# lizaibeim/mmla-audio

Measured on AMD Instinct MI355X. Metric: audio clips/sec (MFCC→logits) at 1/2/4/8 MI355X; MFCC max-abs-err vs librosa, higher is better.
Workload: dtype f16x3+f32

## Files before the change

mmla_audio_amd/csrc/context.cpp:

```cpp
#include <algorithm>
#include <cstdarg>
#include <cstdio>
#include <cstdlib>

#include "internal.h"

using namespace mmla;

namespace mmla __attribute__((visibility("hidden"))) {

int fail(mmla_ctx* c, int code, const char* fmt, ...) {
  char buf[512];
  va_list ap;
  va_start(ap, fmt);
  vsnprintf(buf, sizeof(buf), fmt, ap);
  va_end(ap);
  if (c) c->err = buf;
  return code;
}

static hipEvent_t prof_event(mmla_ctx* c) {
  if (!c->prof_pool.empty()) {
    hipEvent_t e = c->prof_pool.back();
    c->prof_pool.pop_back();
// ... 105 lines not shown
                      side ? "trailing" : "leading", side ? i : g - i);
    }
  }
  return MMLA_OK;
}

int finish(mmla_ctx* c, bool dev) {
  HIPCHK(c, hipGetLastError());
  bool guarded = false;
  for (size_t g : c->ws_guard) guarded |= g != 0;
  if (!dev || guarded) HIPCHK(c, hipStreamSynchronize(c->stream));
  if (guarded) return ws_check_guards(c);
  return MMLA_OK;
}

constexpr double kOdBytesPerClip = 3.0 * 128 * 151 * 32 * 4 + 128 * 151 * 3 + 128 * 151 * 4 +
                                   19 * 128 * 4 + 512 * 4 + 64;
constexpr double kSiBytesPerClip = 4.0 * 256 * 32 * 4 + 256 * 39 * 4 + 8 * 128 * 4 + 512 * 4 +
                                   1024 * 4 + 64;

int64_t microbatch(mmla_ctx* c, bool od) {
  const int64_t user = od ? c->od_mb : c->si_mb;
  if (user > 0) return user;
  const int64_t cap = od ? c->od_mb_cap : c->si_mb_cap;
  size_t fr = 0, tot = 0;
  if (hipMemGetInfo(&fr, &tot) != hipSuccess) {
    (void)hipGetLastError();
    return cap;
  }
  double held = 0;
  for (size_t i = 0; i < c->ws_size.size(); ++i)
// ... 17 lines not shown
    {"MMLA_NO_SIFIN", &mmla_ctx::sifin, nullptr},
    {"MMLA_NO_SIPAIR", &mmla_ctx::sipair, nullptr},
    {"MMLA_NO_SICHAIN", &mmla_ctx::sichain, nullptr},
    {"MMLA_NO_LSTM_SPLIT", &mmla_ctx::lstm_split, nullptr},
    {"MMLA_LSTM_SPLIT_MAX", nullptr, &mmla_ctx::lstm_split_max},
    {"MMLA_DEBUG_LSTM_SPIN", nullptr, &mmla_ctx::lstm_spin},
    {"MMLA_DEBUG_TRACE_GUARD", nullptr, &mmla_ctx::debug_trace_guard},
    {"MMLA_NO_SIPAD", &mmla_ctx::si_pad_feat, nullptr},
    {"MMLA_NO_ODU", &mmla_ctx::odu, nullptr},
    {"MMLA_NO_ODW", &mmla_ctx::odw, nullptr},
    {"MMLA_NO_VADW", &mmla_ctx::vadw, nullptr},
    {"MMLA_VADW", nullptr, &mmla_ctx::vadw_all},
    {"MMLA_RB_TILE", &mmla_ctx::rbs, nullptr},
    {"MMLA_NO_RBS_W1L", &mmla_ctx::rbs_w1l, nullptr},
    {"MMLA_NO_RBS_TAILPAIR", &mmla_ctx::rbs_tailpair, nullptr},
    {"MMLA_NO_PIN_OUT", &mmla_ctx::pin_small, nullptr},
};

extern "C" {

int mmla_abi_version(void) { return MMLA_ABI_VERSION; }

int mmla_create(int device, mmla_ctx** out) {
  if (!out) return MMLA_E_INVALID;
  *out = nullptr;
  int ndev = 0;
  if (hipGetDeviceCount(&ndev) != hipSuccess || ndev == 0) return MMLA_E_HIP;
  if (device < 0 || device >= ndev) return MMLA_E_INVALID;
  if (hipSetDevice(device) != hipSuccess) return MMLA_E_HIP;
  mmla_ctx* c = new mmla_ctx();
// ... 190 lines not shown
```

mmla_audio_amd/csrc/internal.h:

```cpp
#pragma once
#include <hip/hip_runtime.h>

#include <cstdint>
#include <cstring>
#include <string>
#include <vector>

#include "../../include/mmla.h"
#include "nr.h"
#include "od_fe.h"
#include "mix.h"
#include "si_fe.h"
#include "ssim.h"
#include "vad.h"

namespace mmla __attribute__((visibility("hidden"))) {

constexpr int OD_H = 128, OD_W = 151, OD_PIX = OD_H * OD_W;
constexpr int OD_IMG = OD_PIX * 3;
constexpr int SI_T = 256, SI_D = 39;
constexpr int SI_NEED_SAMPLES = 160 * 259 + 400;
constexpr int CH[9] = {32, 32, 32, 64, 64, 64, 128, 128, 128};
constexpr bool POOL[9] = {true, false, false, true, false, false, true, false, false};

// ... 99 lines not shown
  int debug_trace_guard = 0;
  int precision = MMLA_PREC_F16X3;
  bool siu = true;
  bool sipu = true;
  bool sifin = true;
  bool sipair = true;
  bool sichain = true;
  bool si_pad_feat = true;
  bool odu = true;
  bool odw = true;
  bool vadw = true;
  int vadw_all = 0;
  bool rbs = true;
  bool rbs_w1l = true;
  bool rbs_tailpair = true;
  bool lstm_split = true;
  int lstm_split_max = 128;
  int lstm_spin = 0;
  int* range_dev = nullptr;
  int* range_host = nullptr;
  bool pin_small = true;
  int* range_map = nullptr;
  int* range_map_dev = nullptr;
  char* pin_out = nullptr;
  char* pin_out_dev = nullptr;
  char* pin_in = nullptr;
  int64_t lstm_split_reruns = 0;
  int64_t range_reruns = 0;
  bool od_f32_only = false, si_f32_only = false;
  bool si_base_f16_bad = false;
// ... 124 lines not shown
  int* timeout = nullptr;
  bool h3() const { return prec == MMLA_PREC_F16X3; }
};
inline Arith unguarded(const mmla_ctx* c) { return Arith{c->precision, c->lstm_split}; }

struct OdGate {
  const int32_t* lens = nullptr;
  int clip_len = -1;
  uint8_t* silent = nullptr;
  const float* ssim = nullptr;
  float ssim_threshold = 0.0f;
};

int run_od_net(mmla_ctx* c, const Arith& ar, const uint8_t* img_u8, const float* img_f32, int64_t n,
               float* probs, int32_t* argmax, OdGate gate = OdGate(), int stop = -1,
               const float** tap = nullptr, int64_t* tap_n = nullptr);
int run_si_net(mmla_ctx* c, const Arith& ar, const float* x, int64_t n, float* probs, int32_t* argmax,
               const uint8_t* silent, int ldx = SI_D, int stop = -1, const float** tap = nullptr,
               int64_t* tap_n = nullptr);

}
```

mmla_audio_amd/csrc/net_runners.cpp:

```cpp
#include <algorithm>

#include "conv.h"
#include "conv_h3.h"
#include "internal.h"
#include "nets.h"
#include "odu.h"
#include "resblk.h"
#include "siu.h"

using namespace mmla;

namespace {

ConvArgs conv_args(const ConvW& w, const float* x, float* y, int n, int h, int wd, int stride,
                   const BnW* bn, int pro, int epi, const float* res) {
  ConvArgs a{};
  a.x = x;
  a.wt = w.wt;
  a.bias = w.bias;
  a.scale = bn ? bn->scale : nullptr;
  a.shift = bn ? bn->shift : nullptr;
  a.res = res;
  a.y = y;
  a.n = n;
// ... 152 lines not shown
    k.path = OD_STRIPS;
    k.w1_lds = c->rbs_w1l && !POOL[b];
    k.tail_pair = c->rbs_tailpair && POOL[b];
  } else if (tiles_ok(B, POOL[b])) {
    k.path = OD_TILES;
  } else if (c->odu && odu_ok(B, POOL[b], h, w)) {
    k.path = OD_ODU;
    k.strips = c->odw && odu_two_strips(h, w, B.ca.cin, B.ca.cout, POOL[b]) ? 2 : 1;
  }
  k.stem = b == 0 && stop != 0 && (k.path == OD_STRIPS || k.path == OD_TILES);
  return k;
}

ResBlkArgs resblk_args(const ResUnitW& B, bool pool, bool fused, const float* x, float* y, int64_t n,
                       int h, int w, int* range_flag, const ConvW* stem, const uint8_t* img_u8,
                       const float* img_f32) {
  ResBlkArgs r{};
  r.x = x;
  r.y = y;
  r.w1h = fused ? B.ca.fh : B.ca.wh;
  r.w1l = fused ? B.ca.fl : B.ca.wl;
  r.b1 = B.ca.bias;
  r.u1 = B.ca.unscale();
  r.s1 = B.bn_in.scale;
  r.t1 = B.bn_in.shift;
  r.w2h = fused ? B.cb.fh : B.cb.wh;
  r.w2l = fused ? B.cb.fl : B.cb.wl;
  r.b2 = B.cb.bias;
  r.u2 = B.cb.unscale();
  r.s2 = B.bn_mid.scale;
  r.t2 = B.bn_mid.shift;
  if (pool) {
    r.wsh = fused ? B.sc.fh : B.sc.wh;
    r.wsl = fused ? B.sc.fl : B.sc.wl;
    r.bs = B.sc.bias;
    r.us = B.sc.unscale();
  }
  if (stem) {
    r.x = nullptr;
    r.img8 = img_u8;
    r.imgf = img_u8 ? nullptr : img_f32;
    r.wst = stem->wt;
    r.bst = stem->bias;
    r.ldst = stem->cout_pad;
  }
  r.n = (int)n;
  r.h = h;
  r.w = w;
  r.range_flag = range_flag;
  return r;
}

OduArgs odu_args(const ResUnitW& B, bool pool, const float* x, float* y, int64_t n, int* range_flag) {
  OduArgs o{};
  o.x = x;
// ... 43 lines not shown
    CHK(conv_spatial(c, ar, B.cb, T1, T2, n, h, w, &B.bn_mid, PRO_BN_ELU, EPI_BIAS, nullptr, true, 0, &B.sc,
                     X));
    std::swap(T1, T2);
  } else {
    CHK(conv_spatial(c, ar, B.cb, T1, T2, n, h, w, &B.bn_mid, PRO_BN_ELU, EPI_BIAS, nullptr, true));
    CHK(conv_run(c, conv_args(B.sc, X, T1, n, h, w, 2, nullptr, PRO_NONE, EPI_ADD, T2)));
  }
  *out = T1;
  return MMLA_OK;
}

}

namespace mmla __attribute__((visibility("hidden"))) {

int run_od_net(mmla_ctx* c, const Arith& ar, const uint8_t* img_u8, const float* img_f32, int64_t n,
               float* probs, int32_t* argmax, OdGate gate, int stop, const float** tap, int64_t* tap_n) {
  const OdNet& W = c->od;
  const size_t big = (size_t)n * OD_PIX * 32;
  float *X, *T1, *T2, *SEQ, *H;
  CHK(ws_floats(c, S_X, big, &X));
  CHK(ws_floats(c, S_T1, big, &T1));
  CHK(ws_floats(c, S_T2, big, &T2));
  CHK(ws_floats(c, S_SEQ, (size_t)n * 19 * 128, &SEQ));
  CHK(ws_floats(c, S_HOUT, (size_t)n * 512, &H));
  const double stem_flops = 2.0 * n * OD_PIX * 3 * 16;
  const OdChoice first = od_choose(c, ar, W.blk[0], 0, OD_H, OD_W, stop);
  if (!first.stem)
    LAUNCH(c, MMLA_STAGE_GLUE, stem_flops,
           od_stem_launch(img_u8, img_f32, n * OD_PIX, W.stem.cout_pad, W.stem.wt, W.stem.bias, X,
                          c->stream));
  int h = OD_H, w = OD_W;
  if (stop == 0) {
    *tap = X;
    *tap_n = n * OD_PIX * 16;
    return MMLA_OK;
  }
  for (int b = 0; b < 9; ++b) {
    const ResUnitW& B = W.blk[b];
    const bool pool = POOL[b];
    const OdChoice k = b == 0 ? first : od_choose(c, ar, B, b, h, w, stop);
    const double flops = od_block_flops(B, pool, n, h, w) + (k.stem ? stem_flops : 0.0);
    float* out = T1;
    switch (k.path) {
      case OD_STRIPS:
      case OD_TILES: {
        const bool tiles = k.path == OD_TILES;
        const ResBlkArgs r = resblk_args(B, pool, tiles, X, T1, n, h, w, ar.range,
                                         k.stem ? &W.stem : nullptr, img_u8, img_f32);
        LAUNCH(c, MMLA_STAGE_CONV, flops,
               tiles ? resblk_launch(r, B.ca.cin, B.ca.cout, pool, c->stream)
                     : rbs_launch(r, B.ca.cin, B.ca.cout, pool, k.w1_lds, k.tail_pair, c->stream));
        break;
      }
      case OD_ODU: {
        const OduArgs o = odu_args(B, pool, X, T1, n, ar.range);
        LAUNCH(c, MMLA_STAGE_CONV, flops,
               odu_launch(o, h, w, B.ca.cin, B.ca.cout, pool, k.strips, c->stream));
        break;
      }
      case OD_PAIR:
        CHK(od_block_pair(c, ar, B, pool, (int)n, h, w, X, T1, T2, &out));
        break;
    }
// ... 213 lines not shown
```

mmla_audio_amd/csrc/od_fe.h:

```cpp
#pragma once
#include <hip/hip_runtime.h>
#include <stdint.h>

struct OdFeTables {
  int mel_start[128];
  int mel_cnt[128];
  float mel_w[128][10];
  uint16_t a1[16][2][2][64][8];
  uint16_t a2[13][2][2][64][8];
  int mel_bt_bin0[8], mel_bt_nk[8], mel_bt_frag[8];
  int mel_unit[16];
  float mel_a[64][64];
  uint16_t zero16;
};

struct OdFeArgs {
  const int16_t* pcm;
  const float* pcm_f32;
  int64_t clip_stride;
  const int32_t* lens;
  int32_t clip_len;
  const OdFeTables* tables;
  float* db;
  float* norm;
  float* zcr;
  uint8_t* img;
  int* range_flag;
};

void od_fe_build_tables(OdFeTables* t);
bool od_fe_tables_ok(const OdFeTables& t);
hipError_t od_fe_launch(const OdFeArgs& a, int64_t n_clips, hipStream_t stream);
```

mmla_audio_amd/csrc/od_fe.hip:

```cpp
#include "common.h"
#include "od_fe.h"

#include <algorithm>
#include <cstdlib>
#include <cstring>
#include <type_traits>
#include <utility>

namespace {

constexpr int N_FFT = 400;
constexpr int HOP = 160;
constexpr int CLIP = 24000;
constexpr int NF = 151;
constexpr int NMEL = 128;
namespace v3 {

typedef float f32x16 __attribute__((ext_vector_type(16)));
typedef _Float16 f16x8 __attribute__((ext_vector_type(8)));
typedef uint16_t us2 __attribute__((ext_vector_type(2)));

constexpr int NWV = 16;
constexpr int NTH = 64 * NWV;
constexpr int TF = 32;
// ... 99 lines not shown
MMLA_DEV void for_tiles(F&& f, std::integer_sequence<int, I...>) {
  (f(tile_c<I>{}), ...);
}

#ifndef FE_TRACE
#define FE_TRACE 0
#endif
#if FE_TRACE
__device__ unsigned long long fe_trace_buf[256 * 16 * 5 * 8];
#define FE_T(i) do { if (trace_on) tt[i] = __builtin_amdgcn_s_memtime(); } while (0)
#define FE_TFLUSH(t) do { if (trace_on && lane == 0) { for (int i_ = 0; i_ < 8; ++i_) fe_trace_buf[(((size_t)blockIdx.x * 16 + wid) * 5 + (t)) * 8 + i_] = tt[i_]; } } while (0)
#else
#define FE_T(i) do { } while (0)
#define FE_TFLUSH(t) do { } while (0)
#endif
template <bool DB, bool NM, bool IMG>
__global__ void __launch_bounds__(NTH, 1) od_fe3_kernel(OdFeArgs a, int64_t n_clips) {
  __shared__ __attribute__((aligned(16))) Smem sm;
  const OdFeTables& tb = *a.tables;
  const int tid = threadIdx.x;
  const int lane = tid & 63;
  const int wid = __builtin_amdgcn_readfirstlane(tid >> 6);

  f16x8 a1h[G1][2], a1l[G1][2], a2h[G2][2], a2l[G2][2];
#pragma unroll
  for (int g = 0; g < G1; ++g)
#pragma unroll
    for (int s = 0; s < 2; ++s) {
      a1h[g][s] = *reinterpret_cast<const f16x8*>(tb.a1[G1 * wid + g][s][0][lane]);
      a1l[g][s] = *reinterpret_cast<const f16x8*>(tb.a1[G1 * wid + g][s][1][lane]);
    }
// ... 320 lines not shown
    float mx = sm.red[0][0], mn = sm.red[1][0];
#pragma unroll
    for (int w = 1; w < NWV; ++w) {
      mx = fmaxf(mx, sm.red[0][w]);
      mn = fminf(mn, sm.red[1][w]);
    }
    const float lmx = lg2m(mx);
    const float nref = -(lmx * DB_PER_LOG2);
    const float d_max = fmaf(lmx, DB_PER_LOG2, nref);
    const float thr = d_max - 80.0f;
    const float d_min = fmaxf(fmaf(lg2m(mn), DB_PER_LOG2, nref), thr);
    const float diff = d_max - d_min;
    const float inv_diff = 1.0f / diff;
    const int tz = otid();
    if (a.zcr && tz < NF) a.zcr[clip * NF + tz] = (float)sm.zc[par][tz] * (1.0f / 400.0f);
    constexpr uint32_t FB = NMEL * NF * 4, IB = NMEL * NF * 3;
    const auto rn = wave_rsrc(NM ? a.norm + clip * (NMEL * NF) : nullptr, NM ? FB : 0);
    const auto rd = wave_rsrc(DB ? a.db + clip * (NMEL * NF) : nullptr, DB ? FB : 0);
    const auto ri = wave_rsrc(IMG ? a.img + clip * (NMEL * NF * 3) : nullptr, IMG ? IB : 0);
    int l = lane;
    asm volatile("" : "+v"(l));
    const int fr = 16 * m_fh + (l & 15);
    const uint32_t vf = (uint32_t)(4 * (l >> 4) * NF + (l & 15)) * 4u;
    const int sf = (16 * m_bt * NF + 16 * m_fh) * 4;
    const uint32_t vi = (uint32_t)((12 - 4 * (l >> 4)) * NF + (l & 15)) * 3u;
    const int si = ((112 - 16 * m_bt) * NF + 16 * m_fh) * 3;
#pragma unroll
    for (int t = 0; t < NTILE; ++t) {
      if (TF * t + TF > NF && TF * t + fr >= NF) continue;
      uint32_t rr = 0;
      if (IMG) rr = (uint32_t)(int)(((double)sm.zc[par][TF * t + fr] / 400.0) * 255.0) & 255u;
#pragma unroll
      for (int i = 0; i < 4; ++i) {
        const float d = fmaxf(fmaf(dbv[t][i], DB_PER_LOG2, nref), thr);
        const float nv = (d - d_min) * inv_diff;
        const int so = sf + (i * NF + TF * t) * 4;
        if (NM) __builtin_amdgcn_raw_buffer_store_b32(__builtin_bit_cast(uint32_t, nv), rn, vf, so, 0);
        if (DB) __builtin_amdgcn_raw_buffer_store_b32(__builtin_bit_cast(uint32_t, d), rd, vf, so, 0);
        if (IMG) {
          const double v = (1.0 - (double)nv) * 255.0;
          const uint32_t gb = (v >= 0.0) ? ((uint32_t)(int)v & 255u) : 0u;
          const int soi = si + ((3 - i) * NF + TF * t) * 3;
          __builtin_amdgcn_raw_buffer_store_b8((uint8_t)rr, ri, vi, soi, 0);
          __builtin_amdgcn_raw_buffer_store_b8((uint8_t)gb, ri, vi + 1, soi, 0);
          __builtin_amdgcn_raw_buffer_store_b8((uint8_t)gb, ri, vi + 2, soi, 0);
        }
      }
    }
  };

  const int64_t my_clips = (int64_t)blockIdx.x < n_clips ? (n_clips - 1 - blockIdx.x) / gridDim.x + 1 : 0;
  if (my_clips > 0) {
    prefetch(blockIdx.x, tile_c<0>{});
    stage(blockIdx.x, tile_c<0>{});
    prefetch(blockIdx.x, tile_c<1>{});
  }
  __syncthreads();

#pragma unroll 1
  for (int64_t ci = 0; ci <= my_clips; ++ci) {
// ... 95 lines not shown
  }
  if (frags > v3::MFRAG) return false;
  return true;
}

static void launch_v3(const OdFeArgs& a, int64_t n, hipStream_t s) {
  static int n_cu = [] {
    int dev = 0, v = 0;
    if (hipGetDevice(&dev) != hipSuccess ||
        hipDeviceGetAttribute(&v, hipDeviceAttributeMultiprocessorCount, dev) != hipSuccess || v <= 0)
      v = 256;
    return v;
  }();
  const dim3 g((unsigned)std::min<int64_t>(n, n_cu)), b(v3::NTH);
  const int k = (a.db ? 4 : 0) | (a.norm ? 2 : 0) | (a.img ? 1 : 0);
  switch (k) {
    case 0: hipLaunchKernelGGL((v3::od_fe3_kernel<false, false, false>), g, b, 0, s, a, n); break;
    case 1: hipLaunchKernelGGL((v3::od_fe3_kernel<false, false, true>), g, b, 0, s, a, n); break;
    case 2: hipLaunchKernelGGL((v3::od_fe3_kernel<false, true, false>), g, b, 0, s, a, n); break;
    case 3: hipLaunchKernelGGL((v3::od_fe3_kernel<false, true, true>), g, b, 0, s, a, n); break;
    case 4: hipLaunchKernelGGL((v3::od_fe3_kernel<true, false, false>), g, b, 0, s, a, n); break;
    case 5: hipLaunchKernelGGL((v3::od_fe3_kernel<true, false, true>), g, b, 0, s, a, n); break;
    case 6: hipLaunchKernelGGL((v3::od_fe3_kernel<true, true, false>), g, b, 0, s, a, n); break;
    default: hipLaunchKernelGGL((v3::od_fe3_kernel<true, true, true>), g, b, 0, s, a, n); break;
  }
}

hipError_t od_fe_launch(const OdFeArgs& a, int64_t n_clips, hipStream_t stream) {
  if (n_clips <= 0) return hipSuccess;
  launch_v3(a, n_clips, stream);
  return hipGetLastError();
}

void od_fe_build_tables(OdFeTables* t) {
  const double PI = 3.14159265358979323846;
  auto hz_to_mel = [](double f) {
    const double f_sp = 200.0 / 3, min_log_hz = 1000.0, min_log_mel = 1000.0 / f_sp;
    const double logstep = log(6.4) / 27.0;
    return f >= min_log_hz ? min_log_mel + log(f / min_log_hz) / logstep : f / f_sp;
  };
  auto mel_to_hz = [](double m) {
    const double f_sp = 200.0 / 3, min_log_hz = 1000.0, min_log_mel = 1000.0 / f_sp;
    const double logstep = log(6.4) / 27.0;
    return m >= min_log_mel ? min_log_hz * exp(logstep * (m - min_log_mel)) : f_sp * m;
// ... 115 lines not shown
```

mmla_audio_amd/csrc/pipeline.cpp:

```cpp
#include <algorithm>
#include <cmath>
#include <numeric>
#include <type_traits>

#include "internal.h"
#include "resample.h"

using namespace mmla;

namespace {


template <typename T>
struct PcmT {
  const T* p;
  int64_t stride;
  const int32_t* lens;
  int32_t clip_len;
  int32_t true_len;
};
using Pcm = PcmT<int16_t>;

template <typename T>
int stage_pcm(mmla_ctx* c, const T* pcm, int64_t c0, int64_t cnt, int64_t stride,
// ... 262 lines not shown
}

int gate_passes(mmla_ctx* c, const Pcm& p, int64_t cnt, int D, int nr_passes, const int32_t* profile, bool ns,
                float* y0, float* y1, int16_t* q) {
  LAUNCH(c, MMLA_STAGE_GLUE, (double)cnt * D * 6, pcm_f32_launch(p.p, p.stride, p.lens, D, cnt, y0, c->stream));
  for (int k = 0; k < nr_passes; ++k) {
    if (k) HIPCHK(c, hipStreamSynchronize(c->stream));
    CHK(nr_reduce_dev(c, y0, cnt, D, D, y1, profile, ns));
    const bool last = k == nr_passes - 1;
    LAUNCH(c, MMLA_STAGE_GLUE, (double)cnt * D * (last ? 6 : 8),
           requant_launch(y1, p.lens, D, cnt, last ? nullptr : y0, last ? q : nullptr, c->stream));
  }
  return MMLA_OK;
}

int od_image(mmla_ctx* c, const Pcm& p, int64_t cnt, int slot, const uint8_t** img) {
  void* pimg = nullptr;
  CHK(ws_get(c, slot, cnt * OD_IMG, &pimg));
  OdFeArgs a = od_fe_args(c, p);
  a.img = static_cast<uint8_t*>(pimg);
  LAUNCH(c, MMLA_STAGE_OD_FE, od_fe_bytes(cnt, a), od_fe_launch(a, cnt, c->stream));
  *img = a.img;
  return MMLA_OK;
}

int od_net_out(mmla_ctx* c, const Arith& ar, const uint8_t* img, const Pcm& p, OdGate g, int64_t c0, int64_t cnt,
               bool dev, float* probs, int32_t* argmax, uint8_t* silent) {
  float* dp;
  int32_t* da;
  const int k = c->od.k;
  CHK(out_ptr(c, probs, c0 * k, cnt * k, dev, S_OUT0, &dp));
  CHK(out_ptr(c, argmax, c0, cnt, dev, S_OUT1, &da));
  CHK(out_ptr(c, silent, c0, cnt, dev, S_OUT2, &g.silent));
  g.lens = p.lens;
  g.clip_len = p.true_len;
  CHK(run_od_net(c, ar, img, nullptr, cnt, dp, da, g));
  CHK(copy_back(c, probs, c0 * k, dp, cnt * k, dev));
  CHK(copy_back(c, argmax, c0, da, cnt, dev));
  return copy_back(c, silent, c0, g.silent, cnt, dev);
}

int od_fe_net(mmla_ctx* c, const Arith& ar, const Pcm& p, int64_t c0, int64_t cnt, bool dev, float* probs,
              int32_t* argmax, uint8_t* silent) {
  const uint8_t* img;
  CHK(od_image(c, p, cnt, S_IMG, &img));
  return od_net_out(c, ar, img, p, OdGate(), c0, cnt, dev, probs, argmax, silent);
}

int od_pipeline_common(mmla_ctx* c, const int16_t* pcm, int64_t n, int64_t stride, const int32_t* lens,
                       int32_t clip_len, bool gated, int32_t nr_passes, float ssim_threshold,
                       float* probs, int32_t* argmax, uint8_t* silent, float* ssim, uint32_t flags,
                       bool pcm_dev = false) {
  const char* bad = bad_pcm_args(pcm, n, stride, lens, clip_len) ? "bad pcm args" : nullptr;
  const bool ns = flags & MMLA_NR_NONSTATIONARY;
  if (c && !bad && gated) {
    if (nr_passes < 0) bad = "nr_passes < 0";
    else if (nr_passes > 0 && !ns && !c->nr_ready) bad = "nr_passes > 0: mmla_nr_set_noise must be called first";
  }
  return clip_call(c, NET_OD, n, flags, bad, [&](int64_t c0, int64_t cnt, bool dev, const Arith& ar) -> int {
    Pcm p;
    CHK(stage_pcm(c, pcm, c0, cnt, stride, lens, clip_len, MMLA_OD_CLIP, dev || pcm_dev, &p));
// ... 904 lines not shown
```

mmla_audio_amd/csrc/rbs.hip:

```cpp
#define RBS_KERNEL rbs_kernel
#define RBS_W1L false
#include "rbs_body.h"

namespace {

template <int H, int W, int CIN, bool POOL, bool STEM>
hipError_t launch(const ResBlkArgs& a, hipStream_t s) {
  using G = SG<H, W, CIN, POOL>;
  const int64_t blocks = (int64_t)a.n * G::STRIPS;
  if (blocks > 0x7fffffffLL) return hipErrorInvalidValue;
  hipLaunchKernelGGL((rbs_kernel<H, W, CIN, POOL, STEM>), dim3((unsigned)blocks), dim3(NT), 0, s, a);
  return hipGetLastError();
}

}

#if RBS_TRACE
extern "C" int mmla_debug_rbs_trace(unsigned long long* out) {
  return hipMemcpyFromSymbol(out, HIP_SYMBOL(rbs_trace_buf), sizeof(rbs_trace_buf)) == hipSuccess ? 0 : -2;
}
#endif

bool rbs_supported(int h, int w, int cin, int c, bool pool) {
  return c == 32 && ((h == 128 && w == 151 && cin == 16 && pool) || (h == 64 && w == 76 && cin == 32 && !pool));
}

hipError_t rbs_launch(const ResBlkArgs& a, int cin, int c, bool pool, bool w1_lds, bool tail_pair, hipStream_t s) {
  if (a.n == 0) return hipSuccess;
  if (!rbs_supported(a.h, a.w, cin, c, pool) || !a.y || !a.w1h || !a.w1l || !a.w2h || !a.w2l)
    return hipErrorInvalidValue;
  if (pool) {
    if (!a.wsh || !a.wsl || !a.bs) return hipErrorInvalidValue;
    if (a.img8 || a.imgf) return tail_pair ? rbs_tp_launch(a, s) : launch<128, 151, 16, true, true>(a, s);
    return hipErrorInvalidValue;
  }
  if (!a.x || a.x == a.y) return hipErrorInvalidValue;
  return w1_lds ? rbs_w1l_launch(a, s) : launch<64, 76, 32, false, false>(a, s);
}
```

mmla_audio_amd/csrc/rbs_body.h:

```cpp
#pragma once
#include "f16x3.h"
#include "resblk.h"
#if !defined(RBS_KERNEL) || !defined(RBS_W1L)
#error "define RBS_KERNEL and RBS_W1L before including rbs_body.h"
#endif
#ifndef RBS_TAILPAIR
#define RBS_TAILPAIR false
#endif
#ifndef RBS_SC_DEDUP
#define RBS_SC_DEDUP false
#endif

namespace {

constexpr int NT = 256;
constexpr int TW = 16;
constexpr int R = 8;
constexpr int C = 32;
#ifndef RBS_TRACE
#define RBS_TRACE 0
#endif
#if RBS_TRACE
__device__ unsigned long long rbs_trace_buf[2048 * 4 * 4 * 8];
#define RBS_T(i) do { if (bid < 2048 && k >= 2 && k < 6) tt[i] = __builtin_amdgcn_s_memtime(); } while (0)
#define RBS_TFLUSH() do { if (bid < 2048 && k >= 2 && k < 6 && lane == 0) { for (int i_ = 0; i_ < 8; ++i_) rbs_trace_buf[(((size_t)bid * 4 + wave) * 4 + (k - 2)) * 8 + i_] = tt[i_]; } } while (0)
// ... 48 lines not shown
  constexpr int KS1L = W1L ? G::KS1 - 1 : 0;
  static_assert(!W1L || 4 * (G::XPLANE + G::TPLANE + KS1L * 512) + 3 * C * 4 <= 160 * 1024 / 2, "LDS of two workgroups");
  __shared__ __attribute__((aligned(16))) _Float16 sx[2 * G::XPLANE];
  __shared__ __attribute__((aligned(16))) _Float16 st[2 * G::TPLANE];
  __shared__ float4 spar[3 * C / 4 + (STEM ? 16 : 0)];
  __shared__ __attribute__((aligned(16))) _Float16 sw2[G::W2L ? 2 * G::KS2 * 512 : 8];
  __shared__ __attribute__((aligned(16))) _Float16 sw1[W1L ? 2 * KS1L * 512 : 8];

  const int tid = threadIdx.x, lane = tid & 63;
  const int wave = __builtin_amdgcn_readfirstlane(tid >> 6);
  const int h = lane >> 5;
  const uint32_t bid = xcd_block_id();
  constexpr bool TP = RBS_TAILPAIR, SCD = RBS_SC_DEDUP;
  static_assert(!TP || (STEM && W % TW == TW / 2 - 1), "paired tails: block 1, two 7-column tails in one strip");
  static_assert(!SCD || TP, "the de-duplicated shortcut stem belongs to the paired-tails kernel");
  constexpr int FS = TP ? G::STRIPS - 1 : G::STRIPS;
  const bool pair = TP && bid >= (uint32_t)a.n * FS;
  const int clip = pair ? 2 * (int)(bid - (uint32_t)a.n * FS) : (int)(bid / FS);
  const int w0 = pair ? FS * TW : (int)(bid - (uint32_t)clip * FS) * TW;
  const bool has_b = pair && clip + 1 < a.n;
  auto ring_col = [&](int x, int& part, int& iw) -> bool {
    part = TP && pair && x >= G::XW / 2;
    iw = w0 - 1 + x - (TP ? part * (G::XW / 2) : 0);
    return iw >= 0 && iw < W && (!TP || !part || has_b);
  };
  const int lofs = lane * 8;
  float rmax = 0.0f;

  float* const sp = reinterpret_cast<float*>(spar);
  if (tid < C) {
// ... 50 lines not shown
      const float4 v = spar[3 * C / 4 + 4 * q + c];
      bnw[c][0] = s16 * v.x;
      bnw[c][1] = s16 * v.y;
      bnw[c][2] = s16 * v.z;
      bnw[c][3] = fmaf(s16, v.w, t16);
    } else {
      bnw[c][0] = s16;
      bnw[c][1] = t16;
    }
  }

  constexpr uint32_t ROWB = STEM ? 0u : (uint32_t)W * CIN * 4;
  const __amdgpu_buffer_rsrc_t rx = STEM ? w_rsrc(nullptr) :
      __builtin_amdgcn_make_buffer_rsrc(const_cast<float*>(a.x) + (int64_t)clip * H * W * CIN, (short)0,
                                        (int)(H * ROWB), 0x00020000);
  const bool im8 = STEM && a.img8 != nullptr;
  const __amdgpu_buffer_rsrc_t rimg = !STEM ? w_rsrc(nullptr) :
      __builtin_amdgcn_make_buffer_rsrc(im8 ? (void*)(a.img8 + (int64_t)clip * H * W * 3)
                                            : (void*)(a.imgf + (int64_t)clip * H * W * 3),
                                        (short)0, TP ? __builtin_amdgcn_readfirstlane((int)(H * W * 3 * (im8 ? 1 : 4)) * (has_b ? 2 : 1))
                                                     : (int)(H * W * 3 * (im8 ? 1 : 4)), 0x00020000);
  uint32_t tinfo[G::MAXT];
  uint32_t tsrc[TP ? G::MAXT : 1];
#pragma unroll
  for (int j = 0; j < G::MAXT; ++j) {
    const int t = tid + j * NT;
    const int px = t / G::QPP;
    const int rr = px / G::XW, x = px - rr * G::XW;
    int part, iw;
    const bool col_ok = ring_col(x, part, iw);
    const uint32_t tc = !col_ok ? 0u : STEM ? (uint32_t)iw * (a.img8 ? 3u : 12u) : (uint32_t)(iw * CIN + 4 * q) * 4u;
    if constexpr (TP) tsrc[j] = tc + (uint32_t)(part * H * W) * (a.img8 ? 3u : 12u);
    tinfo[j] = (uint32_t)(xoff<CIN>(0, x, q >> 1) + 4 * (q & 1)) | ((uint32_t)(rr & 15) << 10) |
               ((uint32_t)col_ok << 14) | ((uint32_t)(rr < R) << 15) | ((TP ? 0u : tc) << 16);
  }
  auto load_src = [&](int ih, int iw, bool col_ok, int part = 0) -> float4 {
    if constexpr (STEM) {
      const int pix = TP ? (part * H + ih) * W + iw : ih * W + iw;
      const bool ok = col_ok && ih >= 0 && ih < H;
      if (im8) {
        const uint32_t off = ok ? (uint32_t)pix * 3u : 0x80000000u;
        const uint32_t r = __builtin_amdgcn_raw_buffer_load_b8(rimg, off, 0, 0);
        const uint32_t g = __builtin_amdgcn_raw_buffer_load_b8(rimg, off + 1u, 0, 0);
        const uint32_t b = __builtin_amdgcn_raw_buffer_load_b8(rimg, off + 2u, 0, 0);
        return make_float4(__builtin_bit_cast(float, r), __builtin_bit_cast(float, g), __builtin_bit_cast(float, b), 0.f);
      }
      const uint32_t off = ok ? (uint32_t)pix * 12u : 0x80000000u;
      return make_float4(__builtin_bit_cast(float, __builtin_amdgcn_raw_buffer_load_b32(rimg, off, 0, 0)),
                         __builtin_bit_cast(float, __builtin_amdgcn_raw_buffer_load_b32(rimg, off + 4u, 0, 0)),
                         __builtin_bit_cast(float, __builtin_amdgcn_raw_buffer_load_b32(rimg, off + 8u, 0, 0)), 0.f);
    } else {
      const uint32_t off = col_ok ? (uint32_t)ih * ROWB + (uint32_t)(iw * CIN + 4 * q) * 4u : 0x80000000u;
      return __builtin_bit_cast(float4, __builtin_amdgcn_raw_buffer_load_b128(rx, off, 0, 0));
    }
  };
  auto img_px = [&](float4 v) -> float4 {
    if (im8)
      return make_float4((float)__builtin_bit_cast(uint32_t, v.x), (float)__builtin_bit_cast(uint32_t, v.y),
                         (float)__builtin_bit_cast(uint32_t, v.z), 0.f);
    return v;
  };
  auto load_task = [&](int r0, int j) -> float4 {
    const uint32_t ti = tinfo[j];
    const uint32_t off = (ti >> 14) & 1u ? (uint32_t)((r0 + (int)((ti >> 10) & 15)) * (STEM ? W * 3 * (im8 ? 1 : 4) : (int)ROWB)) +
                                               (TP ? tsrc[TP ? j : 0] : ti >> 16)
                                         : 0x80000000u;
    if constexpr (STEM) {
      if (im8) {
        const uint32_t r = __builtin_amdgcn_raw_buffer_load_b8(rimg, off, 0, 0);
        const uint32_t g = __builtin_amdgcn_raw_buffer_load_b8(rimg, off + 1u, 0, 0);
        const uint32_t b = __builtin_amdgcn_raw_buffer_load_b8(rimg, off + 2u, 0, 0);
        return make_float4(__builtin_bit_cast(float, r), __builtin_bit_cast(float, g), __builtin_bit_cast(float, b), 0.f);
      }
      return make_float4(__builtin_bit_cast(float, __builtin_amdgcn_raw_buffer_load_b32(rimg, off, 0, 0)),
                         __builtin_bit_cast(float, __builtin_amdgcn_raw_buffer_load_b32(rimg, off + 4u, 0, 0)),
                         __builtin_bit_cast(float, __builtin_amdgcn_raw_buffer_load_b32(rimg, off + 8u, 0, 0)), 0.f);
    } else {
      return __builtin_bit_cast(float4, __builtin_amdgcn_raw_buffer_load_b128(rx, off, 0, 0));
    }
  };
  auto stage4 = [&](int o, bool in, float4 v, auto MASK_) {
    constexpr bool MASK = decltype(MASK_)::value;
// ... 392 lines not shown
```

mmla_audio_amd/csrc/resblk.h:

```cpp
#pragma once
#include <hip/hip_runtime.h>
#include <stdint.h>

struct ResBlkArgs {
  const float* x;
  const uint16_t* w1h;
  const uint16_t* w1l;
  const float* b1;
  const float* s1;
  const float* t1;
  const uint16_t* w2h;
  const uint16_t* w2l;
  const float* b2;
  const float* s2;
  const float* t2;
  const uint16_t* wsh;
  const uint16_t* wsl;
  const float* bs;
  const uint8_t* img8;
  const float* imgf;
  const float* wst;
  const float* bst;
  int ldst;
  float* y;
  int n, h, w;
  int tiles_h, tiles_w;
  int* range_flag;
  float u1, u2, us;
};

int resblk_k1pad(int cin);
bool resblk_supported(int cin, int c, bool pool);
hipError_t resblk_launch(ResBlkArgs a, int cin, int c, bool pool, hipStream_t stream);
void resblk_split_weights(const float* w, int taps, int cin, int cout, int kpad, uint16_t* hi,
                          uint16_t* lo, bool frag, float wscale);

bool rbs_supported(int h, int w, int cin, int c, bool pool);
hipError_t rbs_launch(const ResBlkArgs& a, int cin, int c, bool pool, bool w1_lds, bool tail_pair,
                      hipStream_t stream);
hipError_t rbs_w1l_launch(const ResBlkArgs& a, hipStream_t stream);
hipError_t rbs_tp_launch(const ResBlkArgs& a, hipStream_t stream);
```

mmla_audio_amd/csrc/resblk.hip:

```cpp
#include "f16x3.h"
#include "resblk.h"

#define RB_MARK(k)

#include <algorithm>
#include <cstring>

namespace {

typedef float f32x4 __attribute__((ext_vector_type(4)));

constexpr int NT = 256;
constexpr int TW = 16;
constexpr int TH = 16;
constexpr int TH_NP = 16;
constexpr float ACT_RANGE = SPLIT_MAX / ACT_SCALE;

typedef float f32x2 __attribute__((ext_vector_type(2)));
typedef _Float16 f16x2 __attribute__((ext_vector_type(2)));
constexpr float LOG2E = 1.4426950408889634f;

__device__ __forceinline__ f32x2 elu2(f32x2 u) {
  const f32x2 t = u * LOG2E;
  f32x2 e = {__builtin_amdgcn_exp2f(t.x), __builtin_amdgcn_exp2f(t.y)};
// ... 537 lines not shown
  return hipGetLastError();
}

}


int resblk_k1pad(int cin) { return (9 * cin + 31) / 32 * 32; }

bool resblk_supported(int cin, int c, bool pool) {
  return c == 32 && ((cin == 16 && pool) || (cin == 32 && !pool));
}

hipError_t resblk_launch(ResBlkArgs a, int cin, int c, bool pool, hipStream_t s) {
  if ((int64_t)a.n * a.h * a.w == 0) return hipSuccess;
  if (!resblk_supported(cin, c, pool)) return hipErrorInvalidValue;
  const int th = pool ? TH : TH_NP;
  a.tiles_h = (a.h + th - 1) / th;
  a.tiles_w = (a.w + TW - 1) / TW;
  if ((int64_t)a.n * a.tiles_h * a.tiles_w > 0x7fffffffLL) return hipErrorInvalidValue;
  if (cin == 16) {
    if (a.img8 || a.imgf) return launch<16, 32, true, true>(a, s);
    return launch<16, 32, true>(a, s);
  }
  return launch<32, 32, false>(a, s);
}

static uint16_t f16_bits(float f) {
  _Float16 h = (_Float16)f;
  uint16_t b;
  memcpy(&b, &h, 2);
// ... 19 lines not shown
```

Measured before the change: 177,400.

## Pack OD spectrogram image as 32-bit pixels between front-end and stem block

Adds a 4-byte-per-pixel layout for the intermediate OD image. The front-end kernel writes one 32-bit store per pixel instead of three byte stores, and a new paired-tails stem kernel variant reads one 32-bit load per pixel instead of three byte loads. The goal is fewer memory instructions on both sides of the image handoff, at the cost of a third more image bytes and a new kernel instantiation. It is gated on the strips/tail-pair path being selected and can be disabled by an environment switch.

```diff
diff --git a/mmla_audio_amd/csrc/context.cpp b/mmla_audio_amd/csrc/context.cpp
--- a/mmla_audio_amd/csrc/context.cpp
+++ b/mmla_audio_amd/csrc/context.cpp
@@ -143,7 +143,7 @@
   return MMLA_OK;
 }
 
-constexpr double kOdBytesPerClip = 3.0 * 128 * 151 * 32 * 4 + 128 * 151 * 3 + 128 * 151 * 4 +
+constexpr double kOdBytesPerClip = 3.0 * 128 * 151 * 32 * 4 + 128 * 151 * 4 + 128 * 151 * 4 +
                                    19 * 128 * 4 + 512 * 4 + 64;
 constexpr double kSiBytesPerClip = 4.0 * 256 * 32 * 4 + 256 * 39 * 4 + 8 * 128 * 4 + 512 * 4 +
                                    1024 * 4 + 64;
@@ -191,6 +191,7 @@
     {"MMLA_RB_TILE", &mmla_ctx::rbs, nullptr},
     {"MMLA_NO_RBS_W1L", &mmla_ctx::rbs_w1l, nullptr},
     {"MMLA_NO_RBS_TAILPAIR", &mmla_ctx::rbs_tailpair, nullptr},
+    {"MMLA_NO_IMG32", &mmla_ctx::img32, nullptr},
     {"MMLA_NO_PIN_OUT", &mmla_ctx::pin_small, nullptr},
 };
 
diff --git a/mmla_audio_amd/csrc/internal.h b/mmla_audio_amd/csrc/internal.h
--- a/mmla_audio_amd/csrc/internal.h
+++ b/mmla_audio_amd/csrc/internal.h
@@ -137,6 +137,7 @@
   bool rbs = true;
   bool rbs_w1l = true;
   bool rbs_tailpair = true;
+  bool img32 = true;
   bool lstm_split = true;
   int lstm_split_max = 128;
   int lstm_spin = 0;
@@ -291,7 +292,8 @@
 
 int run_od_net(mmla_ctx* c, const Arith& ar, const uint8_t* img_u8, const float* img_f32, int64_t n,
                float* probs, int32_t* argmax, OdGate gate = OdGate(), int stop = -1,
-               const float** tap = nullptr, int64_t* tap_n = nullptr);
+               const float** tap = nullptr, int64_t* tap_n = nullptr, int img_px = 3);
+bool od_px32_ok(const mmla_ctx* c, const Arith& ar);
 int run_si_net(mmla_ctx* c, const Arith& ar, const float* x, int64_t n, float* probs, int32_t* argmax,
                const uint8_t* silent, int ldx = SI_D, int stop = -1, const float** tap = nullptr,
                int64_t* tap_n = nullptr);
diff --git a/mmla_audio_amd/csrc/net_runners.cpp b/mmla_audio_amd/csrc/net_runners.cpp
--- a/mmla_audio_amd/csrc/net_runners.cpp
+++ b/mmla_audio_amd/csrc/net_runners.cpp
@@ -190,7 +190,7 @@
 
 ResBlkArgs resblk_args(const ResUnitW& B, bool pool, bool fused, const float* x, float* y, int64_t n,
                        int h, int w, int* range_flag, const ConvW* stem, const uint8_t* img_u8,
-                       const float* img_f32) {
+                       const float* img_f32, int img_px) {
   ResBlkArgs r{};
   r.x = x;
   r.y = y;
@@ -215,6 +215,7 @@
   if (stem) {
     r.x = nullptr;
     r.img8 = img_u8;
+    r.img_px = img_u8 ? img_px : 0;
     r.imgf = img_u8 ? nullptr : img_f32;
     r.wst = stem->wt;
     r.bst = stem->bias;
@@ -288,9 +289,17 @@
 
 namespace mmla __attribute__((visibility("hidden"))) {
 
+bool od_px32_ok(const mmla_ctx* c, const Arith& ar) {
+  const OdChoice k = od_choose(c, ar, c->od.blk[0], 0, OD_H, OD_W, -1);
+  return k.path == OD_STRIPS && k.tail_pair && k.stem;
+}
+
 int run_od_net(mmla_ctx* c, const Arith& ar, const uint8_t* img_u8, const float* img_f32, int64_t n,
-               float* probs, int32_t* argmax, OdGate gate, int stop, const float** tap, int64_t* tap_n) {
+               float* probs, int32_t* argmax, OdGate gate, int stop, const float** tap, int64_t* tap_n,
+               int img_px) {
   const OdNet& W = c->od;
+  if (img_px != 3 && !(img_px == 4 && img_u8 && stop < 0 && od_px32_ok(c, ar)))
+    return fail(c, MMLA_E_INVALID, "run_od_net: %d-byte pixels have no reader in this configuration", img_px);
   const size_t big = (size_t)n * OD_PIX * 32;
   float *X, *T1, *T2, *SEQ, *H;
   CHK(ws_floats(c, S_X, big, &X));
@@ -321,7 +330,7 @@
       case OD_TILES: {
         const bool tiles = k.path == OD_TILES;
         const ResBlkArgs r = resblk_args(B, pool, tiles, X, T1, n, h, w, ar.range,
-                                         k.stem ? &W.stem : nullptr, img_u8, img_f32);
+                                         k.stem ? &W.stem : nullptr, img_u8, img_f32, b == 0 ? img_px : 3);
         LAUNCH(c, MMLA_STAGE_CONV, flops,
                tiles ? resblk_launch(r, B.ca.cin, B.ca.cout, pool, c->stream)
                      : rbs_launch(r, B.ca.cin, B.ca.cout, pool, k.w1_lds, k.tail_pair, c->stream));
diff --git a/mmla_audio_amd/csrc/od_fe.h b/mmla_audio_amd/csrc/od_fe.h
--- a/mmla_audio_amd/csrc/od_fe.h
+++ b/mmla_audio_amd/csrc/od_fe.h
@@ -20,6 +20,7 @@
   int64_t clip_stride;
   const int32_t* lens;
   int32_t clip_len;
+  int32_t img_px;
   const OdFeTables* tables;
   float* db;
   float* norm;
diff --git a/mmla_audio_amd/csrc/od_fe.hip b/mmla_audio_amd/csrc/od_fe.hip
--- a/mmla_audio_amd/csrc/od_fe.hip
+++ b/mmla_audio_amd/csrc/od_fe.hip
@@ -137,7 +137,7 @@
 #define FE_T(i) do { } while (0)
 #define FE_TFLUSH(t) do { } while (0)
 #endif
-template <bool DB, bool NM, bool IMG>
+template <bool DB, bool NM, bool IMG, bool PX32 = false>
 __global__ void __launch_bounds__(NTH, 1) od_fe3_kernel(OdFeArgs a, int64_t n_clips) {
   __shared__ __attribute__((aligned(16))) Smem sm;
   const OdFeTables& tb = *a.tables;
@@ -488,17 +488,19 @@
     const float inv_diff = 1.0f / diff;
     const int tz = otid();
     if (a.zcr && tz < NF) a.zcr[clip * NF + tz] = (float)sm.zc[par][tz] * (1.0f / 400.0f);
-    constexpr uint32_t FB = NMEL * NF * 4, IB = NMEL * NF * 3;
+    static_assert(!PX32 || (IMG && !DB && !NM), "the packed image is the pipeline's only output");
+    constexpr uint32_t IPX = PX32 ? 4 : 3;
+    constexpr uint32_t FB = NMEL * NF * 4, IB = NMEL * NF * IPX;
     const auto rn = wave_rsrc(NM ? a.norm + clip * (NMEL * NF) : nullptr, NM ? FB : 0);
     const auto rd = wave_rsrc(DB ? a.db + clip * (NMEL * NF) : nullptr, DB ? FB : 0);
-    const auto ri = wave_rsrc(IMG ? a.img + clip * (NMEL * NF * 3) : nullptr, IMG ? IB : 0);
+    const auto ri = wave_rsrc(IMG ? a.img + clip * (NMEL * NF * IPX) : nullptr, IMG ? IB : 0);
     int l = lane;
     asm volatile("" : "+v"(l));
     const int fr = 16 * m_fh + (l & 15);
     const uint32_t vf = (uint32_t)(4 * (l >> 4) * NF + (l & 15)) * 4u;
     const int sf = (16 * m_bt * NF + 16 * m_fh) * 4;
-    const uint32_t vi = (uint32_t)((12 - 4 * (l >> 4)) * NF + (l & 15)) * 3u;
-    const int si = ((112 - 16 * m_bt) * NF + 16 * m_fh) * 3;
+    const uint32_t vi = (uint32_t)((12 - 4 * (l >> 4)) * NF + (l & 15)) * IPX;
+    const int si = ((112 - 16 * m_bt) * NF + 16 * m_fh) * (int)IPX;
 #pragma unroll
     for (int t = 0; t < NTILE; ++t) {
       if (TF * t + TF > NF && TF * t + fr >= NF) continue;
@@ -514,10 +516,14 @@
         if (IMG) {
           const double v = (1.0 - (double)nv) * 255.0;
           const uint32_t gb = (v >= 0.0) ? ((uint32_t)(int)v & 255u) : 0u;
-          const int soi = si + ((3 - i) * NF + TF * t) * 3;
-          __builtin_amdgcn_raw_buffer_store_b8((uint8_t)rr, ri, vi, soi, 0);
-          __builtin_amdgcn_raw_buffer_store_b8((uint8_t)gb, ri, vi + 1, soi, 0);
-          __builtin_amdgcn_raw_buffer_store_b8((uint8_t)gb, ri, vi + 2, soi, 0);
+          const int soi = si + ((3 - i) * NF + TF * t) * (int)IPX;
+          if constexpr (PX32) {
+            __builtin_amdgcn_raw_buffer_store_b32(rr | gb << 8 | gb << 16, ri, vi, soi, 0);
+          } else {
+            __builtin_amdgcn_raw_buffer_store_b8((uint8_t)rr, ri, vi, soi, 0);
+            __builtin_amdgcn_raw_buffer_store_b8((uint8_t)gb, ri, vi + 1, soi, 0);
+            __builtin_amdgcn_raw_buffer_store_b8((uint8_t)gb, ri, vi + 2, soi, 0);
+          }
         }
       }
     }
@@ -643,6 +649,10 @@
   }();
   const dim3 g((unsigned)std::min<int64_t>(n, n_cu)), b(v3::NTH);
   const int k = (a.db ? 4 : 0) | (a.norm ? 2 : 0) | (a.img ? 1 : 0);
+  if (a.img_px == 4) {
+    hipLaunchKernelGGL((v3::od_fe3_kernel<false, false, true, true>), g, b, 0, s, a, n);
+    return;
+  }
   switch (k) {
     case 0: hipLaunchKernelGGL((v3::od_fe3_kernel<false, false, false>), g, b, 0, s, a, n); break;
     case 1: hipLaunchKernelGGL((v3::od_fe3_kernel<false, false, true>), g, b, 0, s, a, n); break;
@@ -657,6 +667,8 @@
 
 hipError_t od_fe_launch(const OdFeArgs& a, int64_t n_clips, hipStream_t stream) {
   if (n_clips <= 0) return hipSuccess;
+  if (a.img_px != 0 && a.img_px != 3 && !(a.img_px == 4 && a.img && !a.db && !a.norm && ((uintptr_t)a.img & 3) == 0))
+    return hipErrorInvalidValue;
   launch_v3(a, n_clips, stream);
   return hipGetLastError();
 }
diff --git a/mmla_audio_amd/csrc/pipeline.cpp b/mmla_audio_amd/csrc/pipeline.cpp
--- a/mmla_audio_amd/csrc/pipeline.cpp
+++ b/mmla_audio_amd/csrc/pipeline.cpp
@@ -300,18 +300,19 @@
   return MMLA_OK;
 }
 
-int od_image(mmla_ctx* c, const Pcm& p, int64_t cnt, int slot, const uint8_t** img) {
+int od_image(mmla_ctx* c, const Pcm& p, int64_t cnt, int slot, const uint8_t** img, int img_px = 3) {
   void* pimg = nullptr;
-  CHK(ws_get(c, slot, cnt * OD_IMG, &pimg));
+  CHK(ws_get(c, slot, cnt * OD_PIX * img_px, &pimg));
   OdFeArgs a = od_fe_args(c, p);
   a.img = static_cast<uint8_t*>(pimg);
+  a.img_px = img_px;
   LAUNCH(c, MMLA_STAGE_OD_FE, od_fe_bytes(cnt, a), od_fe_launch(a, cnt, c->stream));
   *img = a.img;
   return MMLA_OK;
 }
 
 int od_net_out(mmla_ctx* c, const Arith& ar, const uint8_t* img, const Pcm& p, OdGate g, int64_t c0, int64_t cnt,
-               bool dev, float* probs, int32_t* argmax, uint8_t* silent) {
+               bool dev, float* probs, int32_t* argmax, uint8_t* silent, int img_px = 3) {
   float* dp;
   int32_t* da;
   const int k = c->od.k;
@@ -320,7 +321,7 @@
   CHK(out_ptr(c, silent, c0, cnt, dev, S_OUT2, &g.silent));
   g.lens = p.lens;
   g.clip_len = p.true_len;
-  CHK(run_od_net(c, ar, img, nullptr, cnt, dp, da, g));
+  CHK(run_od_net(c, ar, img, nullptr, cnt, dp, da, g, -1, nullptr, nullptr, img_px));
   CHK(copy_back(c, probs, c0 * k, dp, cnt * k, dev));
   CHK(copy_back(c, argmax, c0, da, cnt, dev));
   return copy_back(c, silent, c0, g.silent, cnt, dev);
@@ -328,9 +329,10 @@
 
 int od_fe_net(mmla_ctx* c, const Arith& ar, const Pcm& p, int64_t c0, int64_t cnt, bool dev, float* probs,
               int32_t* argmax, uint8_t* silent) {
+  const int img_px = c->img32 && od_px32_ok(c, ar) ? 4 : 3;
   const uint8_t* img;
-  CHK(od_image(c, p, cnt, S_IMG, &img));
-  return od_net_out(c, ar, img, p, OdGate(), c0, cnt, dev, probs, argmax, silent);
+  CHK(od_image(c, p, cnt, S_IMG, &img, img_px));
+  return od_net_out(c, ar, img, p, OdGate(), c0, cnt, dev, probs, argmax, silent, img_px);
 }
 
 int od_pipeline_common(mmla_ctx* c, const int16_t* pcm, int64_t n, int64_t stride, const int32_t* lens,
diff --git a/mmla_audio_amd/csrc/rbs.hip b/mmla_audio_amd/csrc/rbs.hip
--- a/mmla_audio_amd/csrc/rbs.hip
+++ b/mmla_audio_amd/csrc/rbs.hip
@@ -31,6 +31,7 @@
     return hipErrorInvalidValue;
   if (pool) {
     if (!a.wsh || !a.wsl || !a.bs) return hipErrorInvalidValue;
+    if (a.img_px == 4) return tail_pair && a.img8 ? rbs_tp32_launch(a, s) : hipErrorInvalidValue;
     if (a.img8 || a.imgf) return tail_pair ? rbs_tp_launch(a, s) : launch<128, 151, 16, true, true>(a, s);
     return hipErrorInvalidValue;
   }
diff --git a/mmla_audio_amd/csrc/rbs_body.h b/mmla_audio_amd/csrc/rbs_body.h
--- a/mmla_audio_amd/csrc/rbs_body.h
+++ b/mmla_audio_amd/csrc/rbs_body.h
@@ -9,6 +9,9 @@
 #endif
 #ifndef RBS_SC_DEDUP
 #define RBS_SC_DEDUP false
+#endif
+#ifndef RBS_IMG32
+#define RBS_IMG32 false
 #endif
 
 namespace {
@@ -87,6 +90,8 @@
   constexpr bool TP = RBS_TAILPAIR, SCD = RBS_SC_DEDUP;
   static_assert(!TP || (STEM && W % TW == TW / 2 - 1), "paired tails: block 1, two 7-column tails in one strip");
   static_assert(!SCD || TP, "the de-duplicated shortcut stem belongs to the paired-tails kernel");
+  constexpr bool IM32 = RBS_IMG32;
+  static_assert(!IM32 || TP, "the 32-bit pixel image belongs to the paired-tails kernel");
   constexpr int FS = TP ? G::STRIPS - 1 : G::STRIPS;
   const bool pair = TP && bid >= (uint32_t)a.n * FS;
   const int clip = pair ? 2 * (int)(bid - (uint32_t)a.n * FS) : (int)(bid / FS);
@@ -167,8 +172,10 @@
   const __amdgpu_buffer_rsrc_t rx = STEM ? w_rsrc(nullptr) :
       __builtin_amdgcn_make_buffer_rsrc(const_cast<float*>(a.x) + (int64_t)clip * H * W * CIN, (short)0,
                                         (int)(H * ROWB), 0x00020000);
-  const bool im8 = STEM && a.img8 != nullptr;
+  const bool im8 = STEM && (IM32 || a.img8 != nullptr);
   const __amdgpu_buffer_rsrc_t rimg = !STEM ? w_rsrc(nullptr) :
+      IM32 ? __builtin_amdgcn_make_buffer_rsrc((void*)(a.img8 + (int64_t)clip * H * W * 4), (short)0,
+                                               __builtin_amdgcn_readfirstlane((int)(H * W * 4) * (has_b ? 2 : 1)), 0x00020000) :
       __builtin_amdgcn_make_buffer_rsrc(im8 ? (void*)(a.img8 + (int64_t)clip * H * W * 3)
                                             : (void*)(a.imgf + (int64_t)clip * H * W * 3),
                                         (short)0, TP ? __builtin_amdgcn_readfirstlane((int)(H * W * 3 * (im8 ? 1 : 4)) * (has_b ? 2 : 1))
@@ -182,8 +189,8 @@
     const int rr = px / G::XW, x = px - rr * G::XW;
     int part, iw;
     const bool col_ok = ring_col(x, part, iw);
-    const uint32_t tc = !col_ok ? 0u : STEM ? (uint32_t)iw * (a.img8 ? 3u : 12u) : (uint32_t)(iw * CIN + 4 * q) * 4u;
-    if constexpr (TP) tsrc[j] = tc + (uint32_t)(part * H * W) * (a.img8 ? 3u : 12u);
+    const uint32_t tc = !col_ok ? 0u : STEM ? (uint32_t)iw * (IM32 ? 4u : a.img8 ? 3u : 12u) : (uint32_t)(iw * CIN + 4 * q) * 4u;
+    if constexpr (TP) tsrc[j] = tc + (uint32_t)(part * H * W) * (IM32 ? 4u : a.img8 ? 3u : 12u);
     tinfo[j] = (uint32_t)(xoff<CIN>(0, x, q >> 1) + 4 * (q & 1)) | ((uint32_t)(rr & 15) << 10) |
                ((uint32_t)col_ok << 14) | ((uint32_t)(rr < R) << 15) | ((TP ? 0u : tc) << 16);
   }
@@ -191,6 +198,10 @@
     if constexpr (STEM) {
       const int pix = TP ? (part * H + ih) * W + iw : ih * W + iw;
       const bool ok = col_ok && ih >= 0 && ih < H;
+      if constexpr (IM32) {
+        const uint32_t off = ok ? (uint32_t)pix * 4u : 0x80000000u;
+        return make_float4(__builtin_bit_cast(float, __builtin_amdgcn_raw_buffer_load_b32(rimg, off, 0, 0)), 0.f, 0.f, 0.f);
+      }
       if (im8) {
         const uint32_t off = ok ? (uint32_t)pix * 3u : 0x80000000u;
         const uint32_t r = __builtin_amdgcn_raw_buffer_load_b8(rimg, off, 0, 0);
@@ -208,6 +219,10 @@
     }
   };
   auto img_px = [&](float4 v) -> float4 {
+    if constexpr (IM32) {
+      const uint32_t p = __builtin_bit_cast(uint32_t, v.x);
+      return make_float4((float)(p & 255u), (float)((p >> 8) & 255u), (float)((p >> 16) & 255u), 0.f);
+    }
     if (im8)
       return make_float4((float)__builtin_bit_cast(uint32_t, v.x), (float)__builtin_bit_cast(uint32_t, v.y),
                          (float)__builtin_bit_cast(uint32_t, v.z), 0.f);
@@ -215,10 +230,12 @@
   };
   auto load_task = [&](int r0, int j) -> float4 {
     const uint32_t ti = tinfo[j];
-    const uint32_t off = (ti >> 14) & 1u ? (uint32_t)((r0 + (int)((ti >> 10) & 15)) * (STEM ? W * 3 * (im8 ? 1 : 4) : (int)ROWB)) +
+    const uint32_t off = (ti >> 14) & 1u ? (uint32_t)((r0 + (int)((ti >> 10) & 15)) * (IM32 ? W * 4 : STEM ? W * 3 * (im8 ? 1 : 4) : (int)ROWB)) +
                                                (TP ? tsrc[TP ? j : 0] : ti >> 16)
                                          : 0x80000000u;
     if constexpr (STEM) {
+      if constexpr (IM32)
+        return make_float4(__builtin_bit_cast(float, __builtin_amdgcn_raw_buffer_load_b32(rimg, off, 0, 0)), 0.f, 0.f, 0.f);
       if (im8) {
         const uint32_t r = __builtin_amdgcn_raw_buffer_load_b8(rimg, off, 0, 0);
         const uint32_t g = __builtin_amdgcn_raw_buffer_load_b8(rimg, off + 1u, 0, 0);
diff --git a/mmla_audio_amd/csrc/rbs_tp32.hip b/mmla_audio_amd/csrc/rbs_tp32.hip
--- /dev/null
+++ b/mmla_audio_amd/csrc/rbs_tp32.hip
@@ -0,0 +1,15 @@
+#define RBS_KERNEL rbs_tp32_kernel
+#define RBS_W1L false
+#define RBS_TAILPAIR true
+#define RBS_SC_DEDUP true
+#define RBS_IMG32 true
+#include "rbs_body.h"
+
+hipError_t rbs_tp32_launch(const ResBlkArgs& a, hipStream_t s) {
+  using G = SG<128, 151, 16, true>;
+  if (!a.img8 || ((uintptr_t)a.img8 & 3) != 0) return hipErrorInvalidValue;
+  const int64_t blocks = (int64_t)a.n * (G::STRIPS - 1) + (a.n + 1) / 2;
+  if (blocks > 0x7fffffffLL) return hipErrorInvalidValue;
+  hipLaunchKernelGGL((rbs_tp32_kernel<128, 151, 16, true, true>), dim3((unsigned)blocks), dim3(NT), 0, s, a);
+  return hipGetLastError();
+}
diff --git a/mmla_audio_amd/csrc/resblk.h b/mmla_audio_amd/csrc/resblk.h
--- a/mmla_audio_amd/csrc/resblk.h
+++ b/mmla_audio_amd/csrc/resblk.h
@@ -22,6 +22,7 @@
   const float* wst;
   const float* bst;
   int ldst;
+  int img_px;
   float* y;
   int n, h, w;
   int tiles_h, tiles_w;
@@ -40,3 +41,4 @@
                       hipStream_t stream);
 hipError_t rbs_w1l_launch(const ResBlkArgs& a, hipStream_t stream);
 hipError_t rbs_tp_launch(const ResBlkArgs& a, hipStream_t stream);
+hipError_t rbs_tp32_launch(const ResBlkArgs& a, hipStream_t stream);
diff --git a/mmla_audio_amd/csrc/resblk.hip b/mmla_audio_amd/csrc/resblk.hip
--- a/mmla_audio_amd/csrc/resblk.hip
+++ b/mmla_audio_amd/csrc/resblk.hip
@@ -575,6 +575,7 @@
 hipError_t resblk_launch(ResBlkArgs a, int cin, int c, bool pool, hipStream_t s) {
   if ((int64_t)a.n * a.h * a.w == 0) return hipSuccess;
   if (!resblk_supported(cin, c, pool)) return hipErrorInvalidValue;
+  if (a.img_px == 4) return hipErrorInvalidValue;
   const int th = pool ? TH : TH_NP;
   a.tiles_h = (a.h + th - 1) / th;
   a.tiles_w = (a.w + TW - 1) / TW;
```

Result: no change. 178,700 (median of 6 runs) (+0.7%).
